# YaoFANGUK/video-subtitle-remover

Hardware: AMD Instinct MI355X
Metric: inpainted frames/sec @1080p (STTN, 5-frame window) (higher is better)
Workload: dtype f32; 1 GPU; 1080p synthetic clip, --inpaint-mode sttn-auto, 50-frame chunks resident in HBM, neighbor stride 5 / refs every 10 (BASELINE.json metric; model cost is resolution-independent); chunk_frames=50, parallelism=chunk-parallel x1, weights=synthetic variance-preserving (no checkpoint in the reference mount)

## Files before the change

### include/vsr_hip.h

```cpp
#ifndef VSR_HIP_H
#define VSR_HIP_H
#include <stdint.h>

#ifdef __cplusplus
extern "C" {
#endif

#define VSR_OK 0
#define VSR_ERR_ARG (-1)
#define VSR_ERR_STATE (-2)
#define VSR_ERR_HIP (-3)
#define VSR_ERR_NOGPU (-4)

#define VSR_VARIANT_STTN_AUTO 0
#define VSR_VARIANT_STTN_DET 1

typedef struct vsr_sttn vsr_sttn_t;
typedef struct vsr_plan vsr_plan_t;

int vsr_version(void);
const char* vsr_last_error(void);
int vsr_device_count(void);

int vsr_sttn_create(int variant, vsr_sttn_t** out);
// ... 304 lines not shown
    int32_t bufS, bufP;
    int64_t offS, offP, splitStride;
    int32_t M, N, ldS, ldP, nsplit;
    float scale;
} VsrSoftmaxInfo;

int vsr_plan_create(const vsr_sttn_t* h, int L, vsr_plan_t** out);
int vsr_plan_create_rows(const vsr_sttn_t* h, int L, int row_lo, int row_hi, vsr_plan_t** out);
int vsr_plan_create_box(const vsr_sttn_t* h, int L, int row_lo, int row_hi, int col_lo, int col_hi, vsr_plan_t** out);
int vsr_plan_create_ctx(const vsr_sttn_t* h, int L, int n_ctx, int row_lo, int row_hi, int col_lo, int col_hi, vsr_plan_t** out);
int vsr_raft_plan_create(const vsr_raft_t* h, int t, int H, int W, int iters, vsr_plan_t** out);
int vsr_rfc_plan_create(const vsr_rfc_t* h, int t, int H, int W, vsr_plan_t** out);
int vsr_pp_imgprop_plan_create(int t, int H, int W, vsr_plan_t** out);
int vsr_pp_gen_plan_create(const vsr_pp_t* h, int t, int lt, int H, int W, const uint8_t* window_flags, int nflags, vsr_plan_t** out);
int vsr_pp_gen_plan_create_mode(const vsr_pp_t* h, int t, int lt, int H, int W, const uint8_t* window_flags, int nflags, int row_lo, int row_hi,
                                int col_lo, int col_hi, int mode, vsr_plan_t** out);
int vsr_pp_gen_plan_create_box(const vsr_pp_t* h, int t, int lt, int H, int W, const uint8_t* window_flags, int nflags, int row_lo, int row_hi,
                               int col_lo, int col_hi, vsr_plan_t** out);
int vsr_lama_plan_create(const vsr_lama_t* h, int B, int H, int W, vsr_plan_t** out);
int64_t vsr_plan_consts(const vsr_plan_t* p, float* out, int64_t capacity);
void vsr_plan_destroy(vsr_plan_t* p);
int vsr_plan_num_buffers(const vsr_plan_t* p);
int64_t vsr_plan_buffer_elems(const vsr_plan_t* p, int buf);
int vsr_plan_num_tables(const vsr_plan_t* p);
int64_t vsr_plan_table_len(const vsr_plan_t* p, int t);
int vsr_plan_table_copy(const vsr_plan_t* p, int t, int32_t* out);
int vsr_plan_num_ops(const vsr_plan_t* p);
int vsr_plan_op(const vsr_plan_t* p, int i, VsrOpInfo* out);
int vsr_plan_op_lane(const vsr_plan_t* p, int i);
int vsr_plan_op_gemm(const vsr_plan_t* p, int i, int j, VsrGemmInfo* out);
int vsr_plan_op_softmax(const vsr_plan_t* p, int i, int j, VsrSoftmaxInfo* out);
int vsr_plan_counts(const vsr_plan_t* p, int32_t* counts);
double vsr_plan_flops(const vsr_plan_t* p);

#ifdef __cplusplus
}
#endif
#endif
```

### video-subtitle-remover_amd/_lib.py

```python
import ctypes as C
import os

_HERE = os.path.dirname(os.path.abspath(__file__))
LIB_PATH = os.path.join(_HERE, "lib", "libvsr_hip.so")

VSR_OK, VSR_ERR_ARG, VSR_ERR_STATE, VSR_ERR_HIP, VSR_ERR_NOGPU = 0, -1, -2, -3, -4
VARIANT = {"auto": 0, "det": 1}
BMODE_NK, BMODE_KN = 0, 1
ACT_NONE, ACT_LRELU02 = 0, 1
TILE_128x128, TILE_256x32, TILE_256x64, TILE_128x64 = 0, 1, 2, 3
TILE_256x128, TILE_256x256 = 4, 5
TILE_DIMS = {TILE_128x128: (128, 128), TILE_256x32: (256, 32), TILE_256x64: (256, 64), TILE_128x64: (128, 64), TILE_256x128: (256, 128), TILE_256x256: (256, 256)}


class VsrError(RuntimeError):
    def __init__(self, code, msg):
        super().__init__(f"libvsr_hip error {code}: {msg}")
        self.code = code


class GGProblem(C.Structure):
    _fields_ = [("A", C.c_void_p), ("B", C.c_void_p), ("C", C.c_void_p), ("bias", C.c_void_p), ("R", C.c_void_p),
                ("rowA", C.c_void_p), ("colA", C.c_void_p), ("rowB", C.c_void_p), ("colB", C.c_void_p),
                ("rowC", C.c_void_p), ("colC", C.c_void_p), ("rowR", C.c_void_p),
# ... 173 lines not shown
    "vsr_lama_packed_weights": (_L, [_P, _P, _L]),
    "vsr_lama_inpaint": (_I, [_P, _P, _L, _P, _L, _I, _I, _I, _P, _L, _P]),
    "vsr_lama_set_precision": (_I, [_P, _I]),
    "vsr_lama_fallbacks": (_L, [_P]),
    "vsr_lama_read_buffer": (_I, [_P, _I, _L, _L, _P]),
    "vsr_lama_flops": (_D, [_P, _I, _I, _I]),
    "vsr_lama_plan_create": (_I, [_P, _I, _I, _I, C.POINTER(_P)]),
    "vsr_telea_create": (_I, [C.POINTER(_P), _I, _I]),
    "vsr_telea_destroy": (None, [_P]),
    "vsr_telea_set_mask": (_I, [_P, _P, _I, _I]),
    "vsr_telea_plan_pixels": (_L, [_P]),
    "vsr_telea_plan_levels": (_I, [_P]),
    "vsr_telea_plan_taps": (_I, [_P]),
    "vsr_telea_plan_read": (_I, [_P, _P, _P, _P, _P]),
    "vsr_telea_plan_tmap": (_I, [_P, _P]),
    "vsr_telea_plan_weights": (_I, [_P, _P, _P]),
    "vsr_telea_inpaint": (_I, [_P, _P, _L, _I, _P]),
    "vsr_feather_alpha": (_I, [_P, _I, _I, _I, _P, _P]),
    "vsr_feather_composite": (_I, [_P, _L, _P, _L, _P, _I, _I, _I, _I, _P]),
    "vsr_plan_consts": (_L, [_P, _P, _L]),
    "vsr_plan_destroy": (None, [_P]),
    "vsr_plan_num_buffers": (_I, [_P]),
    "vsr_plan_buffer_elems": (_L, [_P, _I]),
    "vsr_plan_num_tables": (_I, [_P]),
    "vsr_plan_table_len": (_L, [_P, _I]),
    "vsr_plan_table_copy": (_I, [_P, _I, _P]),
    "vsr_plan_num_ops": (_I, [_P]),
    "vsr_plan_op": (_I, [_P, _I, C.POINTER(VsrOpInfo)]),
    "vsr_plan_op_lane": (_I, [_P, _I]),
    "vsr_plan_op_gemm": (_I, [_P, _I, _I, C.POINTER(VsrGemmInfo)]),
    "vsr_plan_op_softmax": (_I, [_P, _I, _I, C.POINTER(VsrSoftmaxInfo)]),
    "vsr_plan_counts": (_I, [_P, _P]),
    "vsr_plan_flops": (_D, [_P]),
    "vsr_switch_state": (_I, [C.c_char_p]),
    "vsr_flow_timing": (_I, [_I]),
    "vsr_flow_timing_reset": (_I, []),
    "vsr_flow_timing_get": (_I, [C.c_char_p, C.POINTER(C.c_double), C.POINTER(C.c_int64), C.POINTER(C.c_double)]),
    "vsr_flow_timing_keys": (C.c_int64, [_P, C.c_int64]),
}

if not os.path.exists(LIB_PATH):
    raise ImportError(
        f"{LIB_PATH} is missing: build the HIP extension first (__graft_entry__.build() or "
        f"`make -C {os.path.join(_HERE, 'csrc')}`); this package has no CPU fallback")

import torch

from . import switches

switches.export_defaults()
lib = C.CDLL(LIB_PATH)
for _name, (_res, _args) in SIGNATURES.items():
    _fn = getattr(lib, _name)
    _fn.restype = _res
    _fn.argtypes = _args


def last_error():
    return (lib.vsr_last_error() or b"").decode("utf-8", "replace")


def check(rc):
    if rc != 0:
        raise VsrError(rc, last_error())
    return rc
```

### video-subtitle-remover_amd/csrc/sttn_engine.hip

```cpp
#include <hip/hip_runtime.h>
#include <algorithm>
#include <math.h>
#include <stdio.h>
#include <stdlib.h>
#include <string.h>
#include <map>
#include <memory>
#include <string>
#include <utility>
#include <vector>
#include "../../include/vsr_hip.h"
#include "elementwise.h"
#include "gather_gemm.h"
#include "sttn_plan.h"

using namespace vsr;

static thread_local std::string g_err;
static int fail(int code, const std::string& msg)
{
    g_err = msg;
    return code;
}
int vsr_internal_fail(int code, const char* msg) { return fail(code, msg); }
// ... 9 lines not shown
        int rc_ = (expr);                                                                                  \
        if (rc_ != 0) return rc_;                                                                          \
    } while (0)

namespace {

struct OpDev {
    int kind = 0, tileCfg = 0, bmode = 0;
    const void* dDesc = nullptr;
    int nitems = 0, total = 0;
    int nQueues = 1;
    const void* dDesc7 = nullptr;
    int nitems7 = 0, total7 = 0;
    struct Vt { const float* B; const int32_t* rowB; const int32_t* colB; int K, N; int64_t ld; float* dst; };
    std::vector<Vt> vts;
    const void* src = nullptr;
    void* dst = nullptr;
    int H = 0, W = 0, C = 0, haloS = 0, haloD = 0, n = 0, ldy = 0, pix = 0, premask = 0;
    const int32_t* tFrameIdx = nullptr;
    const int32_t* tFirst = nullptr;
    const uint8_t* maskU8 = nullptr;
    const uint8_t* inU8 = nullptr;
    int M = 0, N = 0, nsplit = 0;
    int64_t splitStride = 0;
    const int32_t* tRowC = nullptr;
    const int32_t* tColC = nullptr;
    int rowLo = 0, rowHi = 0;
    int split = 0;
    bool aexp = false;
    bool thin = false;
    const float* lsum = nullptr;
    int ldL = 0;
    double flops = 0;
    int lane = 0;
    std::string tag;
};

struct PlanDev {
    std::unique_ptr<Plan> plan;
    uint64_t lastUse = 0;
    int32_t* dTables = nullptr;
    void* dDescs = nullptr;
    int32_t* dIsFloat = nullptr;
    unsigned int* dQueues = nullptr;
    int32_t* dTables7 = nullptr;
    float* dVt = nullptr;
    std::vector<OpDev> ops;
    ~PlanDev()
    {
        if (dTables7) (void)hipFree(dTables7);
        if (dVt) (void)hipFree(dVt);
        if (dQueues) (void)hipFree(dQueues);
        if (dTables) (void)hipFree(dTables);
        if (dDescs) (void)hipFree(dDescs);
        if (dIsFloat) (void)hipFree(dIsFloat);
    }
};

struct StripTables {
    void* dev = nullptr;
    const int32_t *dxofs, *dyofs, *uxofs, *uyofs;
    const int16_t *dialpha, *dibeta, *uialpha, *uibeta;
    const float *ufalpha, *ufbeta;
};

struct TimingRec {
    std::string tag, kernel;
    double flops;
    hipEvent_t a, b;
};

}

static bool sttn_thin(int precision, int bmode, const std::vector<GGProblem>& probs, int totalTiles);

struct vsr_sttn {
    Model model;
    int device = -1;
    bool finalized = false;
    void* bufs[BUF_COUNT] = {};
    int64_t cap[BUF_COUNT] = {};
    std::map<int64_t, std::unique_ptr<PlanDev>> plans;
    uint64_t useClock = 0;
    std::map<std::pair<int, int>, StripTables> strips;
    float* compAreas = nullptr;
    int64_t compAreasCap = 0;
    int32_t* dSel = nullptr;
    int dSelCap = 0;
    int precision = 0;
    float* weightsSplit = nullptr;
    unsigned int* dRangeFlag = nullptr;
    int64_t fallbacks = 0;
    int lanes = 2;
    hipStream_t laneStream[kMaxLanes] = {};
    hipEvent_t evFork = nullptr, evJoin[kMaxLanes] = {};
    std::vector<hipEvent_t> evDecode;
    int timing = 0;
    std::vector<TimingRec> pending;
    std::map<std::string, std::pair<double, std::pair<int, double>>> timed;
    explicit vsr_sttn(int variant) : model(variant)
    {
// ... 83 lines not shown
        if (kSlice < 256 || g.N < 32) return false;
        for (const GemmItem& o : op.gemm)
            if (anchorV7(op, o)) return true;
        return false;
    };
    std::vector<int64_t> vtLane(kMaxLanes, 0);
    int64_t tab7 = 0;
    for (const Op& op : P.ops) {
        if (op.kind != OP_GEMM || op.bmode != VSR_BMODE_KN) continue;
        int64_t sum = 0;
        for (const GemmItem& g : op.gemm)
            if (forV7(op, g)) { sum += (int64_t)g.N * g.K; tab7 += (g.N + 3) / 4 * 4; }
        if (sum > vtLane[op.lane]) vtLane[op.lane] = sum;
    }
    std::vector<int64_t> vtBase(kMaxLanes, 0);
    int64_t vtTotal = 0;
    for (int l = 0; l < kMaxLanes; ++l) { vtBase[l] = vtTotal; vtTotal += (vtLane[l] + 31) / 32 * 32; }
    if (vtTotal > 0) HIPCHK(hipMalloc((void**)&pd->dVt, (size_t)vtTotal * sizeof(float)));
    std::vector<int32_t> hostTab7((size_t)tab7, 0);
    if (tab7 > 0) HIPCHK(hipMalloc((void**)&pd->dTables7, (size_t)tab7 * sizeof(int32_t)));
    int64_t tab7Cursor = 0;
    size_t descBytes = 0;
    for (const Op& op : P.ops) {
        size_t n7 = 0;
        if (op.kind == OP_GEMM) for (const GemmItem& g : op.gemm) if (forV7(op, g)) ++n7;
        descBytes += ((op.gemm.size() + n7) * sizeof(GGProblem) + 63) / 64 * 64 + 64;
        descBytes += (op.softmax.size() * sizeof(SMProblem) + 63) / 64 * 64;
    }
    std::vector<char> hostDesc(descBytes + 64, 0);
    HIPCHK(hipMalloc(&pd->dDescs, descBytes + 64));
    size_t cursor = 0;
    for (const Op& op : P.ops) {
        OpDev od;
        od.kind = op.kind; od.tileCfg = op.tileCfg; od.bmode = op.bmode; od.flops = op.flops; od.tag = op.tag; od.lane = op.lane;
        if (op.kind == OP_GEMM) {
            std::vector<GGProblem> small, big;
            int64_t vtCursor = 0;
            for (size_t j = 0; j < op.gemm.size(); ++j) {
                const GemmItem& g = op.gemm[j];
                GGProblem q{};
                q.A = F(g.bufA, g.offA); q.B = F(g.bufB, g.offB); q.C = F(g.bufC, g.offC);
                if (fmt && g.bufB == BUF_WEIGHTS) q.B = h->weightsSplit + g.offB;
                q.bias = g.offBias >= 0 ? F(g.bufBias, g.offBias) : nullptr;
                q.R = g.bufR >= 0 ? F(g.bufR, g.offR) : nullptr;
                q.rowA = T(g.tRowA); q.colA = T(g.tColA); q.rowB = T(g.tRowB); q.colB = T(g.tColB);
                q.rowC = T(g.tRowC); q.colC = T(g.tColC); q.rowR = T(g.tRowR);
                q.M = g.M; q.N = g.N; q.K = g.K; q.tilesM = g.tilesM; q.tilesN = g.tilesN;
                q.splitK = g.splitK; q.chunksPerSplit = g.chunksPerSplit;
                q.act = g.act | ((fmt && !plainF32(g.bufC)) ? VSR_ACT_OUT_SPLIT : 0);
                q.alpha = g.alpha; q.splitStride = g.splitStride;
                if (forV7(op, g)) {
                    if (op.bmode == VSR_BMODE_KN) {
                        OpDev::Vt vt;
                        vt.B = q.B; vt.rowB = q.rowB; vt.colB = q.colB; vt.K = g.K; vt.N = g.N; vt.ld = g.K;
                        vt.dst = pd->dVt + vtBase[op.lane] + vtCursor;
                        vtCursor += (int64_t)g.N * g.K;
                        for (int n = 0; n < g.N; ++n) hostTab7[(size_t)(tab7Cursor + n)] = (int32_t)((int64_t)n * g.K);
                        q.B = vt.dst; q.rowB = pd->dTables7 + tab7Cursor; q.colB = q.colA;
                        tab7Cursor += (g.N + 3) / 4 * 4;
                        od.vts.push_back(vt);
                    }
                    GGProblem two[2];
                    const int n = vsr_v7_split(&q, cus, two);
                    for (int k = 0; k < n; ++k) big.push_back(two[k]);
                } else {
                    small.push_back(q);
                }
// ... 119 lines not shown
    const int prec = pd->plan->precision;
    const bool persistent = prec ? true : use_persistent();
    if (persistent) HIPCHK(hipMemsetAsync(pd->dQueues, 0, (pd->ops.size() + 1) * 16 * sizeof(unsigned int), stream));
    if (pd->plan->bufElems[BUF_ROWMAX] > 0)
        HIPCHK(hipMemsetAsync(h->bufs[BUF_ROWMAX], 0, (size_t)pd->plan->bufElems[BUF_ROWMAX] * sizeof(unsigned int), stream));
    const bool laned = pd->plan->lanes > 1;
    hipStream_t laneOf[kMaxLanes] = {stream, stream, stream, stream};
    if (laned) {
        if (!h->evFork) HIPCHK(hipEventCreateWithFlags(&h->evFork, hipEventDisableTiming));
        for (int l = 1; l < pd->plan->lanes; ++l) {
            if (!h->laneStream[l]) HIPCHK(hipStreamCreateWithFlags(&h->laneStream[l], hipStreamNonBlocking));
            if (!h->evJoin[l]) HIPCHK(hipEventCreateWithFlags(&h->evJoin[l], hipEventDisableTiming));
            laneOf[l] = h->laneStream[l];
        }
    }
    bool forked[kMaxLanes] = {};
    int lastDecodeLane = -1;
    size_t nDecode = 0;
    size_t opIndex = 0;
    for (const OpDev& od : pd->ops) {
        unsigned int* queue = persistent ? pd->dQueues + 16 * opIndex : nullptr;
        if (laned && (int)opIndex == pd->plan->firstWindowOp) HIPCHK(hipEventRecord(h->evFork, laneOf[0]));
        ++opIndex;
        hipStream_t const stream = laneOf[od.lane];
        if (laned && od.lane > 0 && !forked[od.lane]) {
            HIPCHK(hipStreamWaitEvent(stream, h->evFork, 0));
            forked[od.lane] = true;
        }
        if (laned && od.kind == OP_DECODE_OUT && lastDecodeLane >= 0 && lastDecodeLane != od.lane)
            HIPCHK(hipStreamWaitEvent(stream, h->evDecode[nDecode - 1], 0));
        TimingRec tr;
        const bool timed = h->timing == 1 || (h->timing == 2 && od.kind == OP_GEMM && od.tileCfg == VSR_TILE_128x64 && od.bmode == VSR_BMODE_NK && !od.thin);
        if (timed) {
            tr.tag = od.tag; tr.flops = od.flops;
            const bool big = od.kind == OP_GEMM && od.total7 > 0;
            tr.kernel = od.kind != OP_GEMM ? ("kernel:op:" + std::to_string(od.kind))
                      : (big && od.total == 0) ? ("kernel:gg:" + std::to_string(VSR_TILE_256x256) + ":0:v7")
                      : ("kernel:gg:" + std::to_string(od.tileCfg) + ":" + std::to_string(od.bmode) + ":v" +
                         std::to_string(od.thin ? 1 : gg_variant(od.bmode, prec)) + (od.aexp ? "x" : "") + (big ? "m" : ""));
            HIPCHK(hipEventCreate(&tr.a));
            HIPCHK(hipEventCreate(&tr.b));
            HIPCHK(hipEventRecord(tr.a, stream));
        }
        int rc = 0;
        static const bool qkSplit = [] { const char* e = getenv("VSR_F16_QK_SPLIT"); return e && atoi(e) == 1; }();
        const bool scoresSplit = prec == 3 && qkSplit && od.kind == OP_GEMM && od.tag == "attn.qk";
        switch (od.kind) {
        case OP_GEMM:
            for (const OpDev::Vt& vt : od.vts)
                if (rc == 0) rc = vsr_launch_kn_to_nk_split(vt.B, vt.rowB, vt.colB, vt.K, vt.N, vt.ld, vt.dst, stream);
            if (rc == 0 && od.total7 > 0)
                rc = vsr_launch_gather_gemm_dev((const GGProblem*)od.dDesc7, od.nitems7, od.total7, VSR_TILE_256x256, VSR_BMODE_NK, queue + 8,
                                                (prec == 3 && !scoresSplit) ? 6 : 5, 1, h->dRangeFlag, stream);
            if (rc == 0 && od.total > 0)
                rc = vsr_launch_gather_gemm_dev((const GGProblem*)od.dDesc, od.nitems, od.total, od.tileCfg, od.bmode, queue,
                                                (scoresSplit ? 5 : od.thin ? 1 : gg_variant(od.bmode, prec)) | (od.aexp ? VSR_VARIANT_A_EXP : 0), od.nQueues,
                                                prec ? h->dRangeFlag : nullptr, stream);
            break;
        case OP_SOFTMAX:
            rc = vsr_launch_softmax_dev((const SMProblem*)od.dDesc, od.nitems, od.total, stream);
            break;
        case OP_NORM_IM2COL:
            rc = vsr_launch_norm_im2col_fmt((const uint8_t*)od.src, od.H, od.W, od.n, (float*)od.dst, od.premask, od.maskU8, od.split, stream);
            break;
        case OP_UPSAMPLE2X:
            rc = vsr_launch_upsample2x_rows((const float*)od.src, od.H, od.W, od.C, od.haloS, (float*)od.dst, od.haloD, od.n, od.split,
                                            od.rowLo, od.rowHi > od.rowLo ? od.rowHi : 2 * od.H, stream);
// ... 21 lines not shown
        if (laned && od.kind == OP_DECODE_OUT) {
            if (h->evDecode.size() <= nDecode) {
                hipEvent_t e;
                HIPCHK(hipEventCreateWithFlags(&e, hipEventDisableTiming));
                h->evDecode.push_back(e);
            }
            HIPCHK(hipEventRecord(h->evDecode[nDecode], stream));
            lastDecodeLane = od.lane;
            ++nDecode;
        }
    }
    for (int l = 1; l < kMaxLanes; ++l)
        if (forked[l]) {
            HIPCHK(hipEventRecord(h->evJoin[l], laneOf[l]));
            HIPCHK(hipStreamWaitEvent(laneOf[0], h->evJoin[l], 0));
        }
    return 0;
}

static bool switch_rows_on() { static const bool v = [] { const char* e = getenv("VSR_DECODE_ROWS"); return !(e && atoi(e) == 0); }(); return v; }
static bool switch_cols_on() { static const bool v = [] { const char* e = getenv("VSR_DECODE_COLS"); return e && atoi(e) == 1; }(); return v; }

static int collect_timing(vsr_sttn* h, hipStream_t stream)
{
    if (h->pending.empty()) return 0;
    HIPCHK(hipStreamSynchronize(stream));
    for (TimingRec& tr : h->pending) {
        float ms = 0.f;
        HIPCHK(hipEventElapsedTime(&ms, tr.a, tr.b));
        for (const std::string* key : {&tr.tag, &tr.kernel}) {
            auto& acc = h->timed[*key];
            acc.first += ms;
            acc.second.first += 1;
            acc.second.second += tr.flops;
        }
        (void)hipEventDestroy(tr.a);
        (void)hipEventDestroy(tr.b);
    }
    h->pending.clear();
    return 0;
}

static int need_gpu(vsr_sttn* h)
{
    if (!h) return fail(VSR_ERR_ARG, "null handle");
    if (!h->finalized || h->device < 0)
        return fail(VSR_ERR_NOGPU, "model is not finalized on a HIP device (no GPU / finalize(device<0)); there is no CPU fallback");
    HIPCHK(hipSetDevice(h->device));
    return 0;
}

static int get_strip_tables(vsr_sttn* h, int W, int sh, StripTables** out)
{
    auto key = std::make_pair(W, sh);
    auto it = h->strips.find(key);
    if (it != h->strips.end()) { *out = &it->second; return 0; }
    const int mw = h->model.g.modelW, mh = h->model.g.modelH;
    std::vector<int32_t> dxo, dyo, uxo, uyo;
    std::vector<int16_t> dxa, dya, uxa, uya;
    std::vector<float> dxf, dyf, uxf, uyf;
    cv2_linear_tables(W, mw, true, dxo, dxa, dxf);
    cv2_linear_tables(sh, mh, false, dyo, dya, dyf);
    cv2_linear_tables(mw, W, true, uxo, uxa, uxf);
    cv2_linear_tables(mh, sh, false, uyo, uya, uyf);
    auto al = [](size_t v) { return (v + 15) / 16 * 16; };
    size_t o = 0;
    const size_t o_dxo = o; o += al(dxo.size() * 4);
// ... 493 lines not shown

double vsr_sttn_flops(vsr_sttn_t* h, int L)
{
    if (!h || !h->model.packed_ready() || L <= 0) { fail(VSR_ERR_ARG, "bad argument"); return -1.0; }
    try {
        Plan p(h->model, L);
        return p.flops;
    } catch (const std::exception& e) {
        fail(VSR_ERR_ARG, e.what());
        return -1.0;
    }
}

double vsr_sttn_flops_reference(vsr_sttn_t* h, int L)
{
    if (!h || !h->model.packed_ready() || L <= 0) { fail(VSR_ERR_ARG, "bad argument"); return -1.0; }
    try {
        Plan p(h->model, L);
        return p.refFlops;
    } catch (const std::exception& e) {
        fail(VSR_ERR_ARG, e.what());
        return -1.0;
    }
}

int vsr_switch_state(const char* name)
{
    if (!name) return -1;
    const std::string n(name);
    if (n == "VSR_DECODE_ROWS") return switch_rows_on() ? 1 : 0;
    if (n == "VSR_DECODE_COLS") return switch_cols_on() ? 1 : 0;
    if (n == "VSR_QKV0_SHARED") return Tuning::get(0).shareQkv0 ? 1 : 0;
    if (n == "VSR_TRIM_LAST_BLOCK") return Tuning::get(0).trimLastBlock ? 1 : 0;
    return -1;
}

int vsr_sttn_timing(vsr_sttn_t* h, int enable)
{
    if (!h) return fail(VSR_ERR_ARG, "null handle");
    h->timing = enable < 0 ? 0 : (enable > 2 ? 1 : enable);
    return 0;
}

int vsr_sttn_timing_reset(vsr_sttn_t* h)
{
    if (!h) return fail(VSR_ERR_ARG, "null handle");
    h->timed.clear();
    return 0;
}

int vsr_sttn_timing_get(vsr_sttn_t* h, const char* prefix, double* total_ms, int32_t* launches, double* flops)
{
    if (!h || !prefix) return fail(VSR_ERR_ARG, "bad argument");
    double ms = 0, fl = 0;
    int n = 0;
    const size_t pl = strlen(prefix);
    for (const auto& kv : h->timed)
        if (kv.first.compare(0, pl, prefix) == 0) { ms += kv.second.first; n += kv.second.second.first; fl += kv.second.second.second; }
    if (total_ms) *total_ms = ms;
    if (launches) *launches = n;
    if (flops) *flops = fl;
    return 0;
}

static void tile_dims(int cfg, int& BM, int& BN)
{
// ... 252 lines not shown
int vsr_plan_op_lane(const vsr_plan_t* p, int i) { return (p && i >= 0 && i < (int)p->plan->ops.size()) ? p->plan->ops[i].lane : -1; }

int vsr_plan_op_gemm(const vsr_plan_t* p, int i, int j, VsrGemmInfo* o)
{
    if (!p || !o || i < 0 || i >= (int)p->plan->ops.size()) return fail(VSR_ERR_ARG, "bad op");
    const Op& op = p->plan->ops[i];
    if (op.kind != OP_GEMM || j < 0 || j >= (int)op.gemm.size()) return fail(VSR_ERR_ARG, "bad gemm item");
    const GemmItem& g = op.gemm[j];
    o->bufA = g.bufA; o->bufB = g.bufB; o->bufC = g.bufC; o->bufR = g.bufR;
    o->offA = g.offA; o->offB = g.offB; o->offC = g.offC; o->offR = g.offR; o->offBias = g.offBias;
    o->tRowA = g.tRowA; o->tColA = g.tColA; o->tRowB = g.tRowB; o->tColB = g.tColB; o->tRowC = g.tRowC;
    o->tColC = g.tColC; o->tRowR = g.tRowR;
    o->M = g.M; o->N = g.N; o->K = g.K; o->tilesM = g.tilesM; o->tilesN = g.tilesN; o->splitK = g.splitK;
    o->chunksPerSplit = g.chunksPerSplit; o->splitStride = g.splitStride; o->alpha = g.alpha; o->act = g.act;
    return 0;
}
int vsr_plan_op_softmax(const vsr_plan_t* p, int i, int j, VsrSoftmaxInfo* o)
{
    if (!p || !o || i < 0 || i >= (int)p->plan->ops.size()) return fail(VSR_ERR_ARG, "bad op");
    const Op& op = p->plan->ops[i];
    if (op.kind != OP_SOFTMAX || j < 0 || j >= (int)op.softmax.size()) return fail(VSR_ERR_ARG, "bad softmax item");
    const SoftmaxItem& s = op.softmax[j];
    o->bufS = s.bufS; o->bufP = s.bufP; o->offS = s.offS; o->offP = s.offP; o->splitStride = s.splitStride;
    o->M = s.M; o->N = s.N; o->ldS = s.ldS; o->ldP = s.ldP; o->nsplit = s.nsplit; o->scale = s.scale;
    return 0;
}
int vsr_plan_counts(const vsr_plan_t* p, int32_t* counts)
{
    if (!p || !counts) return fail(VSR_ERR_ARG, "bad argument");
    memcpy(counts, p->plan->compCount.data(), p->plan->compCount.size() * sizeof(int32_t));
    return 0;
}
double vsr_plan_flops(const vsr_plan_t* p) { return p ? p->plan->flops : -1.0; }

}
```

### video-subtitle-remover_amd/csrc/sttn_plan.cpp

```cpp
#include "sttn_plan.h"
#include "gather_gemm.h"
#include <assert.h>
#include <math.h>
#include <stdexcept>
#include <stdlib.h>

namespace vsr {

static int envInt(const char* name, int dflt)
{
    const char* v = getenv(name);
    return (v && *v) ? atoi(v) : dflt;
}

const Tuning& Tuning::get(int precision)
{
    static const Tuning t[2] = {
        [] {
            Tuning x;
            x.convTile = envInt("VSR_CONV_TILE", VSR_TILE_128x64);
            if (x.convTile == VSR_TILE_256x128) x.convTile = VSR_TILE_128x64;
            x.qkTile = envInt("VSR_QK_TILE", VSR_TILE_128x64);
            x.qkvTile = envInt("VSR_QKV_TILE", x.convTile);
            x.pvTile = envInt("VSR_PV_TILE", VSR_TILE_128x64);
            x.pvSplitChunks = envInt("VSR_PV_SPLIT_CHUNKS", 50);
            x.convChannelMajor = envInt("VSR_CONV_KORDER", 1);
            x.fuseSoftmax = envInt("VSR_FUSE_SOFTMAX", 1) && envInt("VSR_GG_VARIANT", 3) == 3 && envInt("VSR_PV_VARIANT", 1) == 1;
            x.outConvBlocked = envInt("VSR_OUT_CONV_BLOCKED", 1);
            x.trimLastBlock = envInt("VSR_TRIM_LAST_BLOCK", 1);
            x.shareQkv0 = envInt("VSR_QKV0_SHARED", 0);
            return x;
        }(),
        [] {
            Tuning x;
            x.convTile = envInt("VSR_CONV_TILE", VSR_TILE_128x64);
            x.qkTile = envInt("VSR_QK_TILE", VSR_TILE_128x64);
            x.qkvTile = envInt("VSR_QKV_TILE", x.convTile);
            x.pvTile = envInt("VSR_PV_TILE", VSR_TILE_128x64);
            x.pvSplitChunks = envInt("VSR_PV_SPLIT_CHUNKS", 50);
            x.convChannelMajor = envInt("VSR_CONV_KORDER", 1);
            x.fuseSoftmax = 0;
            x.outConvBlocked = envInt("VSR_OUT_CONV_BLOCKED", 1);
            x.trimLastBlock = envInt("VSR_TRIM_LAST_BLOCK", 1);
            x.shareQkv0 = envInt("VSR_QKV0_SHARED", 0);
            return x;
        }()};
    return t[precision ? 1 : 0];
}

static inline int cdiv(int a, int b) { return (a + b - 1) / b; }
static inline int64_t rup(int64_t a, int64_t b) { return (a + b - 1) / b * b; }

Geometry Geometry::make(int variant)
{
    Geometry g{};
    g.variant = variant;
    g.channels = 256;
    g.blocks = 8;
    g.nscales = 4;
    g.neighborStride = 5;
    g.refLength = 10;
    if (variant == 0) {
        g.modelW = 640; g.modelH = 120;
        const int pw[4] = {80, 32, 10, 5}, ph[4] = {15, 6, 5, 3};
        for (int i = 0; i < 4; ++i) { g.patchW[i] = pw[i]; g.patchH[i] = ph[i]; }
    } else {
        g.modelW = 432; g.modelH = 240;
        const int pw[4] = {108, 36, 18, 9}, ph[4] = {60, 20, 10, 5};
        for (int i = 0; i < 4; ++i) { g.patchW[i] = pw[i]; g.patchH[i] = ph[i]; }
    }
    g.featW = g.modelW / 4;
    g.featH = g.modelH / 4;
    return g;
}

Model::Model(int variant) : g(Geometry::make(variant)) { blk.resize(g.blocks); }

// ... 239 lines not shown
                v.push_back((int32_t)o);
            }
    const int32_t first = v.empty() ? 0 : v[0];
    while ((int64_t)v.size() % padTo) v.push_back(first);
    return table(key, std::move(v));
}

int PlanBuilder::tColsConvHW(const Act& a, int kh, int kw, int dil, int c0, int cin)
{
    if (cin < 0) cin = a.C - c0;
    const std::string key = "CC:" + std::to_string(a.halo) + ":" + std::to_string(a.W) + ":" + std::to_string(a.C) +
                            ":" + std::to_string(kh) + "x" + std::to_string(kw) + ":" + std::to_string(dil) + ":" +
                            std::to_string(c0) + ":" + std::to_string(cin);
    auto it = tableKey_.find(key);
    if (it != tableKey_.end()) return it->second;
    if (a.halo < dil * (kh / 2) || a.halo < dil * (kw / 2)) throw std::runtime_error("activation halo too small for conv");
    if (cin % VSR_GG_KC || c0 % VSR_GG_KC) throw std::runtime_error("conv input channels must be a multiple of 32");
    std::vector<int32_t> v;
    auto off = [&](int ky, int kx, int c) {
        return (int32_t)(((int64_t)(ky - kh / 2) * dil * a.Wp() + (kx - kw / 2) * dil) * a.C + c0 + c);
    };
    if (Tuning::get().convChannelMajor) {
        for (int c = 0; c < cin; c += VSR_GG_KC)
            for (int ky = 0; ky < kh; ++ky)
                for (int kx = 0; kx < kw; ++kx) v.push_back(off(ky, kx, c));
    } else {
        for (int ky = 0; ky < kh; ++ky)
            for (int kx = 0; kx < kw; ++kx)
                for (int c = 0; c < cin; c += VSR_GG_KC) v.push_back(off(ky, kx, c));
    }
    return table(key, std::move(v));
}

int PlanBuilder::tRowsLinear(int count, int ld, int padTo)
{
    const std::string key = "RL:" + std::to_string(count) + ":" + std::to_string(ld) + ":" + std::to_string(padTo);
    auto it = tableKey_.find(key);
    if (it != tableKey_.end()) return it->second;
    std::vector<int32_t> v;
    for (int i = 0; i < count; ++i) { checkFits((int64_t)i * ld); v.push_back((int32_t)((int64_t)i * ld)); }
    while ((int)v.size() % padTo) v.push_back(0);
    return table(key, std::move(v));
}

int PlanBuilder::tColsLinear(int nchunks, int padTo)
{
    const std::string key = "CL:" + std::to_string(nchunks) + ":" + std::to_string(padTo);
    auto it = tableKey_.find(key);
    if (it != tableKey_.end()) return it->second;
    std::vector<int32_t> v;
    for (int i = 0; i < nchunks; ++i) v.push_back(i * VSR_GG_KC);
    while ((int)v.size() < padTo) v.push_back(0);
    return table(key, std::move(v));
}

int Plan::tRowsTokens(int T, int s, int choff, int count, int padTo, int oy0, int oy1, int ox0, int ox1, const std::vector<int>* fids)
{
    const int pw = g.patchW[s], ph = g.patchH[s], ow = g.featW / pw, oh = g.featH / ph, C3 = 3 * g.channels;
    if (oy1 < 0) oy1 = oh;
    if (ox1 < 0) ox1 = ow;
    std::string key = "RT:" + std::to_string(T) + ":" + std::to_string(s) + ":" + std::to_string(choff) + ":" +
                      std::to_string(count) + ":" + std::to_string(padTo) + ":" + std::to_string(oy0) + "-" + std::to_string(oy1) +
                      ":" + std::to_string(ox0) + "-" + std::to_string(ox1);
    if (fids) key += ":f" + idsKey(std::vector<int>(fids->begin(), fids->begin() + T));
    auto it = tableKey_.find(key);
    if (it != tableKey_.end()) return it->second;
// ... 61 lines not shown
    for (int y = 0; y < ph; ++y)
        for (int x = 0; x < pw; ++x)
            for (int c0 = 0; c0 < dk; c0 += VSR_GG_KC) v.push_back((int32_t)(((int64_t)y * a.Wp() + x) * a.C + c0));
    while ((int)v.size() < padTo) v.push_back(0);
    return table(key, std::move(v));
}

static std::vector<int> iota(int n)
{
    std::vector<int> v(n);
    for (int i = 0; i < n; ++i) v[i] = i;
    return v;
}

void Plan::addConv(const char* tag, const Act& in, const std::vector<int>& inIds, const Act& out, int nOut, int ksz,
                   int stride, int dil, const ConvW& w, int act, const Act* res, const std::vector<int>* resIds, int ylo, int yhi,
                   int xlo, int xhi)
{
    if (yhi < 0) yhi = out.H;
    if (xhi < 0) xhi = out.W;
    if (ylo < 0 || yhi > out.H || ylo >= yhi || (stride != 1 && (ylo != 0 || yhi != out.H))) throw std::runtime_error(std::string("conv row range: ") + tag);
    if (xlo < 0 || xhi > out.W || xlo >= xhi || (stride != 1 && (xlo != 0 || xhi != out.W))) throw std::runtime_error(std::string("conv column range: ") + tag);
    const bool rect = xlo != 0 || xhi != out.W;
    const int oh = yhi - ylo, ow = xhi - xlo;
    if (w.K != ksz * ksz * in.C) throw std::runtime_error(std::string("conv K mismatch: ") + tag);
    if ((int)inIds.size() != nOut) throw std::runtime_error("conv frame list mismatch");
    Op op;
    op.kind = OP_GEMM;
    op.tag = tag;
    op.bmode = VSR_BMODE_NK;
    op.tileCfg = pickTile(w.cout);
    int BM, BN;
    tileDims(op.tileCfg, BM, BN);
    GemmItem it{};
    it.M = nOut * oh * ow;
    it.N = w.cout;
    it.K = w.K;
    it.tilesM = cdiv(it.M, BM);
    it.tilesN = cdiv(it.N, BN);
    it.splitK = 1;
    it.chunksPerSplit = it.K / VSR_GG_KC;
    it.splitStride = 0;
    it.alpha = 1.f;
    it.act = act;
    it.bufA = in.buf; it.offA = 0;
    it.tRowA = rect ? tRowsActRect(in, inIds, ylo, yhi, xlo, xhi, BM) : tRowsAct(in, inIds, oh, out.W, stride, BM, (int64_t)ylo * in.Wp() * in.C);
    it.tColA = tColsConv(in, ksz, dil);
    it.bufB = BUF_WEIGHTS; it.offB = w.w;
    it.tRowB = tRowsLinear(it.N, it.K, BN);
    it.tColB = tColsLinear(it.K / VSR_GG_KC, it.K / VSR_GG_KC);
    it.bufC = out.buf; it.offC = 0;
    it.tRowC = rect ? tRowsActRect(out, iota(nOut), ylo, yhi, xlo, xhi, BM) : tRowsAct(out, iota(nOut), oh, out.W, 1, BM, (int64_t)ylo * out.Wp() * out.C);
    it.tColC = tColsLinear(cdiv(it.N, VSR_GG_KC), it.tilesN * BN / VSR_GG_KC);
    it.offBias = w.b;
    if (res) {
        it.bufR = res->buf; it.offR = 0;
        it.tRowR = rect ? tRowsActRect(*res, *resIds, ylo, yhi, xlo, xhi, BM) : tRowsAct(*res, *resIds, oh, out.W, 1, BM, (int64_t)ylo * res->Wp() * res->C);
    } else {
        it.bufR = -1; it.offR = 0; it.tRowR = -1;
    }
    op.flops = 2.0 * it.M * it.N * (double)(ksz * ksz * in.C);
    op.gemm.push_back(it);
    need(out.buf, (int64_t)nOut * out.frameElems());
    flops += op.flops;
    ops.push_back(std::move(op));
}

void Plan::addAttention(int Tq, int T, const BlockW&, int attLo, int attHi, int attXLo, int attXHi, int qkvBuf, const std::vector<int>* fids, int qFirst)
{
    std::vector<int> qf;
    for (int t = 0; t < Tq; ++t) qf.push_back(fids ? (*fids)[qFirst + t] : qFirst + t);
    const std::vector<int>* qfids = qFirst > 0 ? &qf : fids;
    if (qkvBuf < 0) qkvBuf = lb(BUF_QKV);
    if (attHi < 0) attHi = g.featH;
    if (attXHi < 0) attXHi = g.featW;
    const Tuning& tu = tu_;
    const int C = g.channels, dk = C / g.nscales;
    const Act att{lb(BUF_ATT), T, g.featH, g.featW, C, 1};
    Op qk, sm, pv;
    qk.kind = OP_GEMM; qk.tag = "attn.qk"; qk.tileCfg = tu.qkTile; qk.bmode = VSR_BMODE_NK;
    sm.kind = OP_SOFTMAX; sm.tag = "attn.softmax";
    pv.kind = OP_GEMM; pv.tag = "attn.pv"; pv.tileCfg = tu.pvTile; pv.bmode = VSR_BMODE_KN;
    int qBM, qBN, pBM, pBN;
    tileDims(qk.tileCfg, qBM, qBN);
    tileDims(pv.tileCfg, pBM, pBN);
    std::vector<Op> reduces;
    bool pvFused = false;
    int64_t sOff = 0, pOff = 0, partOff = 0, lOff = 0;
    for (int s = g.nscales - 1; s >= 0; --s) {
        const int pw = g.patchW[s], ph = g.patchH[s];
        const int Pn = (g.featW / pw) * (g.featH / ph);
        const int Ntok = T * Pn;
        const int oy0 = attLo / ph, oy1 = cdiv(attHi, ph);
        const int ox0 = attXLo / pw, ox1 = cdiv(attXHi, pw);
        const int Mtok = Tq * (oy1 - oy0) * (ox1 - ox0);
// ... 426 lines not shown
        it.bufC = BUF_QKV0; it.offC = 0;
        it.tRowC = tRowsLinear(it.M, 3 * C, BM);
        it.tColC = tColsLinear(it.N / VSR_GG_KC, it.tilesN * BN / VSR_GG_KC);
        it.offBias = bw.qkv.b;
        it.bufR = -1; it.tRowR = -1;
        op.flops = 2.0 * it.M * (double)it.N * it.K;
        flops += op.flops;
        trimmedFlops_ -= op.flops;
        op.gemm.push_back(it);
        need(BUF_QKV0, (int64_t)it.M * 3 * C);
        ops.push_back(std::move(op));
    }

    std::vector<int32_t> visits(L, 0);
    const int ns = g.neighborStride;
    for (int f = 0; f < L; f += ns) {
        std::vector<int> neighbors, refs;
        for (int i = (f - ns > 0 ? f - ns : 0); i < (f + ns + 1 < L ? f + ns + 1 : L); ++i) neighbors.push_back(i);
        for (int i = 0; i < L; i += g.refLength) {
            bool inN = false;
            for (int n : neighbors) inN |= (n == i);
            if (!inN) refs.push_back(i);
        }
        if (neighbors.back() < nCtx) continue;
        lane_ = nwindows % lanes;
        const size_t first = ops.size();
        if (firstWindowOp < 0) firstWindowOp = (int)first;
        buildWindow(neighbors, refs, visits);
        for (size_t i = first; i < ops.size(); ++i) ops[i].lane = lane_;
    }
    lane_ = 0;
    compCount = visits;
    refFlops = flops + trimmedFlops_;
    if (nCtx > 0) refFlops = Plan(model, L_, precision_, 1, decLo_, decHi_, decXLo_, decXHi_).refFlops;
}

void cv2_linear_tables(int ssize, int dsize, bool clampX, std::vector<int32_t>& ofs, std::vector<int16_t>& icoef,
                       std::vector<float>& fcoef)
{
    const double inv_scale = (double)dsize / (double)ssize;
    const double scale = 1.0 / inv_scale;
    ofs.resize(dsize);
    icoef.resize(2 * (size_t)dsize);
    fcoef.resize(2 * (size_t)dsize);
    for (int d = 0; d < dsize; ++d) {
        float f = (float)((d + 0.5) * scale - 0.5);
        int s = (int)floorf(f);
        f -= (float)s;
        if (clampX) {
            if (s < 0) { f = 0.f; s = 0; }
            if (s >= ssize - 1) { f = 0.f; s = ssize - 1; }
        }
        ofs[d] = s;
        const float c0 = 1.f - f, c1 = f;
        fcoef[2 * d] = c0;
        fcoef[2 * d + 1] = c1;
        auto sat = [](float v) {
            long r = lrintf(v * 2048.f);
            if (r > 32767) r = 32767;
            if (r < -32768) r = -32768;
            return (int16_t)r;
        };
        icoef[2 * d] = sat(c0);
        icoef[2 * d + 1] = sat(c1);
    }
}
// ... 3 lines not shown
```

### video-subtitle-remover_amd/csrc/sttn_plan.h

```cpp
#pragma once
#include <stdint.h>
#include <map>
#include <string>
#include <vector>

namespace vsr {

struct Geometry {
    int variant;
    int modelW, modelH;
    int featW, featH;
    int channels;
    int blocks;
    int nscales;
    int patchW[4], patchH[4];
    int neighborStride;
    int refLength;
    static Geometry make(int variant);
};

struct Tuning {
    int convTile;
    int qkTile;
    int qkvTile;
    int pvTile;
    int pvSplitChunks;
    int convChannelMajor;
    int outConvBlocked;
    int shareQkv0;
    int trimLastBlock;
    int fuseSoftmax;
    static const Tuning& get(int precision = 0);
};

struct ConvW {
    int64_t w = -1, b = -1;
    int cout = 0, K = 0;
};
struct BlockW { ConvW qkv, out, ffn1, ffn2; };

class Model {
public:
    explicit Model(int variant);
    bool set_param(const std::string& name, const float* data, const int64_t* shape, int ndim, std::string& err);
    bool pack(std::string& err);
    bool packed_ready() const { return ready_; }
    Geometry g;
    ConvW enc[4], dec[4];
    ConvW dec4blk;
    static constexpr int kOutBlkH = 2, kOutBlkW = 4;
    std::vector<BlockW> blk;
    std::vector<float> packed;
    static std::vector<std::string> expected_keys(int variant);
private:
    struct Raw { std::vector<float> v; std::vector<int64_t> shape; };
    std::map<std::string, Raw> raw_;
    bool ready_ = false;
    bool pack_conv(const std::string& key, ConvW& cw, int cinPad, std::string& err);
    bool pack_conv_blocked(const std::string& key, ConvW& cw, int bh, int bw, std::string& err);
};

enum BufId {
    BUF_WEIGHTS = 0, BUF_IN_U8, BUF_IM2COL, BUF_E1, BUF_E2, BUF_E3, BUF_FEATS, BUF_X0, BUF_X1, BUF_QKV,
    BUF_S, BUF_P, BUF_ATT, BUF_F1, BUF_UP1, BUF_D1, BUF_D2, BUF_UP2, BUF_D3, BUF_D4, BUF_COMP, BUF_PVPART, BUF_MASK_U8,
// ... 18 lines not shown

enum OpKind { OP_NORM_IM2COL = 0, OP_GEMM = 1, OP_SOFTMAX = 2, OP_UPSAMPLE2X = 3, OP_DECODE_OUT = 4, OP_REDUCE_SCATTER = 5,
              OP_EW = 6  };

struct GemmItem {
    int bufA, bufB, bufC, bufR;
    int64_t offA, offB, offC, offR, offBias;
    int tRowA, tColA, tRowB, tColB, tRowC, tColC, tRowR;
    int M, N, K;
    int tilesM, tilesN, splitK, chunksPerSplit;
    int64_t splitStride;
    float alpha;
    int act;
    int bufBias;
};
struct SoftmaxItem {
    int bufS, bufP;
    int64_t offS, offP, splitStride;
    int M, N, ldS, ldP, nsplit;
    float scale;
};
struct Op {
    int kind = 0;
    int tileCfg = 0, bmode = 0;
    std::vector<GemmItem> gemm;
    std::vector<SoftmaxItem> softmax;
    int bufSrc = -1, bufDst = -1, H = 0, W = 0, C = 0, haloS = 0, haloD = 0, n = 0;
    int ldy = 0, pix = 0, tFrameIdx = -1, tFirst = -1;
    int premask = 0;
    int bufMask = -1;
    int M = 0, N = 0, nsplit = 0, tRowC = -1, tColC = -1;
    int64_t offSrc = 0, offDst = 0, splitStride = 0;
    double flops = 0;
    int lane = 0;
    std::string tag;
    int ew = 0;
    int ibuf[4] = {-1, -1, -1, -1};
    int64_t ioff[4] = {0, 0, 0, 0};
    int ipar[16] = {0, 0, 0, 0, 0, 0, 0, 0, 0, 0, 0, 0, 0, 0, 0, 0};
    float fpar[4] = {0.f, 0.f, 0.f, 0.f};
};

struct Act {
    int buf, n, H, W, C, halo;
    int Hp() const { return H + 2 * halo; }
    int Wp() const { return W + 2 * halo; }
    int64_t frameElems() const { return (int64_t)Hp() * Wp() * C; }
    int64_t pix(int f, int y, int x) const { return (((int64_t)f * Hp() + y + halo) * Wp() + x + halo) * C; }
    int64_t elems() const { return (int64_t)n * frameElems(); }
};

constexpr int BUF_PLAN_CONST = -2;

struct PlanIR {
    std::vector<int64_t> bufElems;
    std::vector<float> consts;
    std::vector<std::vector<int32_t>> tables;
    std::vector<Op> ops;
    std::vector<int32_t> compCount;
    double flops = 0;
    double refFlops = 0;
    virtual ~PlanIR() {}
};

class PlanBuilder : public PlanIR {
protected:
    std::map<std::string, int> tableKey_;
    int table(const std::string& key, std::vector<int32_t>&& v);
    int tRowsAct(const Act& a, const std::vector<int>& ids, int oh, int ow, int stride, int padTo, int64_t add);
    int tRowsActRect(const Act& a, const std::vector<int>& ids, int ylo, int yhi, int xlo, int xhi, int padTo);
    int tColsConvHW(const Act& a, int kh, int kw, int dil, int c0 = 0, int cin = -1);
    int tColsConv(const Act& a, int ksz, int dil) { return tColsConvHW(a, ksz, ksz, dil); }
    int tRowsLinear(int count, int ld, int padTo);
    int tColsLinear(int nchunks, int padTo);
    void need(int buf, int64_t elems);
};

class Plan : public PlanBuilder {
public:
    Plan(const Model& model, int L, int precision = 0, int lanes = 1, int decLo = 0, int decHi = 0, int decXLo = 0, int decXHi = 0, int nCtx = 0);
    static void decoder_bounds(const Geometry& g, int precision, int decLo, int decHi, int decXLo, int decXHi, int* lo, int* hi, int* xlo, int* xhi);
    int decLo = 0, decHi = 0;
    int decXLo = 0, decXHi = 0;
    int L;
    int nCtx = 0;
    int precision;
    int lanes;
    int firstWindowOp = -1;
    Geometry g;
    int nwindows = 0;
private:
    const Model& m_;
    const Tuning& tu_;
    int lane_ = 0;
    bool qkv0_ = false;
    int lb(int buf) const { return laneBuf(buf, lane_); }
    int64_t rowmaxElems_ = 0;
    double trimmedFlops_ = 0;
    int pickTile(int N) const;
    int tRowsTokens(int T, int s, int choff, int count, int padTo, int oy0 = 0, int oy1 = -1, int ox0 = 0, int ox1 = -1,
                    const std::vector<int>* fids = nullptr);
    int tColsPatch(int s, int padTo);
    int tRowsTokensAct(const Act& a, int T, int s, int padTo, int oy0 = 0, int oy1 = -1, int ox0 = 0, int ox1 = -1);
    int tColsPatchAct(const Act& a, int s, int padTo);
    void addConv(const char* tag, const Act& in, const std::vector<int>& inIds, const Act& out, int nOut,
// ... 16 lines not shown
```

### video-subtitle-remover_amd/switches.py

```python
import os

DEFAULTS = {"VSR_DECODE_COLS": "1", "VSR_PP_DECODE_BOX": "1", "VSR_PP_ENC_CACHE": "1", "VSR_QKV0_SHARED": "1"}


def export_defaults():
    for k, v in DEFAULTS.items():
        os.environ.setdefault(k, v)


LIBRARY_SIDE = ("VSR_DECODE_COLS", "VSR_QKV0_SHARED")


def on(name):
    if name in LIBRARY_SIDE:
        from . import _lib

        v = _lib.lib.vsr_switch_state(name.encode())
        if v >= 0:
            return v == 1
    return os.environ.get(name, DEFAULTS[name]) == "1"
```

Measured before the change: 220.2 frames/s.

## Skip zero-padding conv taps on top/bottom border rows via split GEMM items

For 3x3 stride-1 convolutions, the output rows are split into a middle band using all nine taps and top/bottom border bands that omit the taps reading only zero-padded halo rows. This shrinks K for the border bands and uses new gather tables for the reduced activation and weight columns. It removes wasted multiply-adds on padding, at the cost of more, smaller GEMM items per op with possible tile underutilization. Executed-FLOP accounting is added for timing reports.

```diff
diff --git a/include/vsr_hip.h b/include/vsr_hip.h
--- a/include/vsr_hip.h
+++ b/include/vsr_hip.h
@@ -360,6 +360,7 @@
 int vsr_plan_op_softmax(const vsr_plan_t* p, int i, int j, VsrSoftmaxInfo* out);
 int vsr_plan_counts(const vsr_plan_t* p, int32_t* counts);
 double vsr_plan_flops(const vsr_plan_t* p);
+double vsr_plan_flops_executed(const vsr_plan_t* p);
 
 #ifdef __cplusplus
 }
diff --git a/video-subtitle-remover_amd/_lib.py b/video-subtitle-remover_amd/_lib.py
--- a/video-subtitle-remover_amd/_lib.py
+++ b/video-subtitle-remover_amd/_lib.py
@@ -229,6 +229,7 @@
     "vsr_plan_op_softmax": (_I, [_P, _I, _I, C.POINTER(VsrSoftmaxInfo)]),
     "vsr_plan_counts": (_I, [_P, _P]),
     "vsr_plan_flops": (_D, [_P]),
+    "vsr_plan_flops_executed": (_D, [_P]),
     "vsr_switch_state": (_I, [C.c_char_p]),
     "vsr_flow_timing": (_I, [_I]),
     "vsr_flow_timing_reset": (_I, []),
diff --git a/video-subtitle-remover_amd/csrc/sttn_engine.hip b/video-subtitle-remover_amd/csrc/sttn_engine.hip
--- a/video-subtitle-remover_amd/csrc/sttn_engine.hip
+++ b/video-subtitle-remover_amd/csrc/sttn_engine.hip
@@ -65,6 +65,7 @@
     const float* lsum = nullptr;
     int ldL = 0;
     double flops = 0;
+    double flopsExec = 0;
     int lane = 0;
     std::string tag;
 };
@@ -99,7 +100,7 @@
 
 struct TimingRec {
     std::string tag, kernel;
-    double flops;
+    double flops, flopsExec;
     hipEvent_t a, b;
 };
 
@@ -249,7 +250,7 @@
     size_t cursor = 0;
     for (const Op& op : P.ops) {
         OpDev od;
-        od.kind = op.kind; od.tileCfg = op.tileCfg; od.bmode = op.bmode; od.flops = op.flops; od.tag = op.tag; od.lane = op.lane;
+        od.kind = op.kind; od.tileCfg = op.tileCfg; od.bmode = op.bmode; od.flops = op.flops; od.flopsExec = op.flopsExecuted >= 0 ? op.flopsExecuted : op.flops; od.tag = op.tag; od.lane = op.lane;
         if (op.kind == OP_GEMM) {
             std::vector<GGProblem> small, big;
             int64_t vtCursor = 0;
@@ -435,7 +436,7 @@
         TimingRec tr;
         const bool timed = h->timing == 1 || (h->timing == 2 && od.kind == OP_GEMM && od.tileCfg == VSR_TILE_128x64 && od.bmode == VSR_BMODE_NK && !od.thin);
         if (timed) {
-            tr.tag = od.tag; tr.flops = od.flops;
+            tr.tag = od.tag; tr.flops = od.flops; tr.flopsExec = od.flopsExec;
             const bool big = od.kind == OP_GEMM && od.total7 > 0;
             tr.kernel = od.kind != OP_GEMM ? ("kernel:op:" + std::to_string(od.kind))
                       : (big && od.total == 0) ? ("kernel:gg:" + std::to_string(VSR_TILE_256x256) + ":0:v7")
@@ -523,7 +524,7 @@
             auto& acc = h->timed[*key];
             acc.first += ms;
             acc.second.first += 1;
-            acc.second.second += tr.flops;
+            acc.second.second += key == &tr.kernel ? tr.flopsExec : tr.flops;
         }
         (void)hipEventDestroy(tr.a);
         (void)hipEventDestroy(tr.b);
@@ -1083,6 +1084,7 @@
     if (n == "VSR_DECODE_COLS") return switch_cols_on() ? 1 : 0;
     if (n == "VSR_QKV0_SHARED") return Tuning::get(0).shareQkv0 ? 1 : 0;
     if (n == "VSR_TRIM_LAST_BLOCK") return Tuning::get(0).trimLastBlock ? 1 : 0;
+    if (n == "VSR_SKIP_PAD_TAPS") return Tuning::get(0).skipPadTaps ? 1 : 0;
     return -1;
 }
 
@@ -1401,5 +1403,6 @@
     return 0;
 }
 double vsr_plan_flops(const vsr_plan_t* p) { return p ? p->plan->flops : -1.0; }
-
-}
+double vsr_plan_flops_executed(const vsr_plan_t* p) { return !p ? -1.0 : (p->plan->flopsExecuted >= 0 ? p->plan->flopsExecuted : p->plan->flops); }
+
+}
diff --git a/video-subtitle-remover_amd/csrc/sttn_plan.cpp b/video-subtitle-remover_amd/csrc/sttn_plan.cpp
--- a/video-subtitle-remover_amd/csrc/sttn_plan.cpp
+++ b/video-subtitle-remover_amd/csrc/sttn_plan.cpp
@@ -1,5 +1,6 @@
 #include "sttn_plan.h"
 #include "gather_gemm.h"
+#include <algorithm>
 #include <assert.h>
 #include <math.h>
 #include <stdexcept>
@@ -29,6 +30,7 @@
             x.outConvBlocked = envInt("VSR_OUT_CONV_BLOCKED", 1);
             x.trimLastBlock = envInt("VSR_TRIM_LAST_BLOCK", 1);
             x.shareQkv0 = envInt("VSR_QKV0_SHARED", 0);
+            x.skipPadTaps = envInt("VSR_SKIP_PAD_TAPS", 1);
             return x;
         }(),
         [] {
@@ -43,6 +45,7 @@
             x.outConvBlocked = envInt("VSR_OUT_CONV_BLOCKED", 1);
             x.trimLastBlock = envInt("VSR_TRIM_LAST_BLOCK", 1);
             x.shareQkv0 = envInt("VSR_QKV0_SHARED", 0);
+            x.skipPadTaps = envInt("VSR_SKIP_PAD_TAPS", 1);
             return x;
         }()};
     return t[precision ? 1 : 0];
@@ -348,6 +351,33 @@
     return table(key, std::move(v));
 }
 
+int PlanBuilder::tColsConvTaps(const Act& a, int dil, unsigned taps)
+{
+    const std::string key = "CT:" + std::to_string(a.halo) + ":" + std::to_string(a.W) + ":" + std::to_string(a.C) + ":" +
+                            std::to_string(dil) + ":" + std::to_string(taps);
+    auto it = tableKey_.find(key);
+    if (it != tableKey_.end()) return it->second;
+    if (a.halo < dil) throw std::runtime_error("activation halo too small for conv");
+    if (a.C % VSR_GG_KC) throw std::runtime_error("conv input channels must be a multiple of 32");
+    std::vector<int32_t> v;
+    for (int c = 0; c < a.C; c += VSR_GG_KC)
+        for (int tap = 0; tap < 9; ++tap)
+            if (taps >> tap & 1) v.push_back((int32_t)(((int64_t)(tap / 3 - 1) * dil * a.Wp() + (tap % 3 - 1) * dil) * a.C + c));
+    return table(key, std::move(v));
+}
+
+int PlanBuilder::tColsWeightTaps(int cin, unsigned taps)
+{
+    const std::string key = "CW:" + std::to_string(cin) + ":" + std::to_string(taps);
+    auto it = tableKey_.find(key);
+    if (it != tableKey_.end()) return it->second;
+    std::vector<int32_t> v;
+    for (int c = 0; c < cin; c += VSR_GG_KC)
+        for (int tap = 0; tap < 9; ++tap)
+            if (taps >> tap & 1) v.push_back((c / VSR_GG_KC * 9 + tap) * VSR_GG_KC);
+    return table(key, std::move(v));
+}
+
 int PlanBuilder::tRowsLinear(int count, int ld, int padTo)
 {
     const std::string key = "RL:" + std::to_string(count) + ":" + std::to_string(ld) + ":" + std::to_string(padTo);
@@ -475,35 +505,54 @@
     op.tileCfg = pickTile(w.cout);
     int BM, BN;
     tileDims(op.tileCfg, BM, BN);
-    GemmItem it{};
-    it.M = nOut * oh * ow;
-    it.N = w.cout;
-    it.K = w.K;
-    it.tilesM = cdiv(it.M, BM);
-    it.tilesN = cdiv(it.N, BN);
-    it.splitK = 1;
-    it.chunksPerSplit = it.K / VSR_GG_KC;
-    it.splitStride = 0;
-    it.alpha = 1.f;
-    it.act = act;
-    it.bufA = in.buf; it.offA = 0;
-    it.tRowA = rect ? tRowsActRect(in, inIds, ylo, yhi, xlo, xhi, BM) : tRowsAct(in, inIds, oh, out.W, stride, BM, (int64_t)ylo * in.Wp() * in.C);
-    it.tColA = tColsConv(in, ksz, dil);
-    it.bufB = BUF_WEIGHTS; it.offB = w.w;
-    it.tRowB = tRowsLinear(it.N, it.K, BN);
-    it.tColB = tColsLinear(it.K / VSR_GG_KC, it.K / VSR_GG_KC);
-    it.bufC = out.buf; it.offC = 0;
-    it.tRowC = rect ? tRowsActRect(out, iota(nOut), ylo, yhi, xlo, xhi, BM) : tRowsAct(out, iota(nOut), oh, out.W, 1, BM, (int64_t)ylo * out.Wp() * out.C);
-    it.tColC = tColsLinear(cdiv(it.N, VSR_GG_KC), it.tilesN * BN / VSR_GG_KC);
-    it.offBias = w.b;
-    if (res) {
-        it.bufR = res->buf; it.offR = 0;
-        it.tRowR = rect ? tRowsActRect(*res, *resIds, ylo, yhi, xlo, xhi, BM) : tRowsAct(*res, *resIds, oh, out.W, 1, BM, (int64_t)ylo * res->Wp() * res->C);
+    auto item = [&](int y0, int y1, unsigned taps) {
+        const int rows = y1 - y0;
+        int ntaps = 0;
+        for (int t = 0; t < ksz * ksz; ++t) ntaps += taps >> t & 1;
+        const bool all = ntaps == ksz * ksz;
+        GemmItem it{};
+        it.M = nOut * rows * ow;
+        it.N = w.cout;
+        it.K = all ? w.K : ntaps * in.C;
+        it.tilesM = cdiv(it.M, BM);
+        it.tilesN = cdiv(it.N, BN);
+        it.splitK = 1;
+        it.chunksPerSplit = it.K / VSR_GG_KC;
+        it.splitStride = 0;
+        it.alpha = 1.f;
+        it.act = act;
+        it.bufA = in.buf; it.offA = 0;
+        it.tRowA = rect ? tRowsActRect(in, inIds, y0, y1, xlo, xhi, BM) : tRowsAct(in, inIds, rows, out.W, stride, BM, (int64_t)y0 * in.Wp() * in.C);
+        it.tColA = all ? tColsConv(in, ksz, dil) : tColsConvTaps(in, dil, taps);
+        it.bufB = BUF_WEIGHTS; it.offB = w.w;
+        it.tRowB = tRowsLinear(it.N, w.K, BN);
+        it.tColB = all ? tColsLinear(it.K / VSR_GG_KC, it.K / VSR_GG_KC) : tColsWeightTaps(in.C, taps);
+        it.bufC = out.buf; it.offC = 0;
+        it.tRowC = rect ? tRowsActRect(out, iota(nOut), y0, y1, xlo, xhi, BM) : tRowsAct(out, iota(nOut), rows, out.W, 1, BM, (int64_t)y0 * out.Wp() * out.C);
+        it.tColC = tColsLinear(cdiv(it.N, VSR_GG_KC), it.tilesN * BN / VSR_GG_KC);
+        it.offBias = w.b;
+        if (res) {
+            it.bufR = res->buf; it.offR = 0;
+            it.tRowR = rect ? tRowsActRect(*res, *resIds, y0, y1, xlo, xhi, BM) : tRowsAct(*res, *resIds, rows, out.W, 1, BM, (int64_t)y0 * res->Wp() * res->C);
+        } else {
+            it.bufR = -1; it.offR = 0; it.tRowR = -1;
+        }
+        op.gemm.push_back(it);
+    };
+    const int H = out.H;
+    if (tu_.skipPadTaps && tu_.convChannelMajor && ksz == 3 && stride == 1 && in.H == H && H >= 2 * dil) {
+        const int topHi = yhi < dil ? yhi : dil, botLo = ylo > H - dil ? ylo : H - dil;
+        const int midLo = ylo > dil ? ylo : dil, midHi = yhi < H - dil ? yhi : H - dil;
+        if (midHi > midLo) item(midLo, midHi, 0x1ff);
+        if (topHi > ylo) item(ylo, topHi, 0x1f8);
+        if (yhi > botLo) item(botLo, yhi, 0x03f);
+        std::stable_sort(op.gemm.begin(), op.gemm.end(), [](const GemmItem& a, const GemmItem& b) { return (int64_t)a.M * a.K > (int64_t)b.M * b.K; });
     } else {
-        it.bufR = -1; it.offR = 0; it.tRowR = -1;
-    }
-    op.flops = 2.0 * it.M * it.N * (double)(ksz * ksz * in.C);
-    op.gemm.push_back(it);
+        item(ylo, yhi, (1u << (ksz * ksz)) - 1);
+    }
+    op.flops = 2.0 * nOut * oh * ow * (double)w.cout * (double)(ksz * ksz * in.C);
+    op.flopsExecuted = 0;
+    for (const GemmItem& it : op.gemm) op.flopsExecuted += 2.0 * it.M * (double)it.N * it.K;
     need(out.buf, (int64_t)nOut * out.frameElems());
     flops += op.flops;
     ops.push_back(std::move(op));
@@ -996,6 +1045,8 @@
     lane_ = 0;
     compCount = visits;
     refFlops = flops + trimmedFlops_;
+    flopsExecuted = 0;
+    for (const Op& op : ops) flopsExecuted += op.flopsExecuted >= 0 ? op.flopsExecuted : op.flops;
     if (nCtx > 0) refFlops = Plan(model, L_, precision_, 1, decLo_, decHi_, decXLo_, decXHi_).refFlops;
 }
 
diff --git a/video-subtitle-remover_amd/csrc/sttn_plan.h b/video-subtitle-remover_amd/csrc/sttn_plan.h
--- a/video-subtitle-remover_amd/csrc/sttn_plan.h
+++ b/video-subtitle-remover_amd/csrc/sttn_plan.h
@@ -30,6 +30,7 @@
     int shareQkv0;
     int trimLastBlock;
     int fuseSoftmax;
+    int skipPadTaps;
     static const Tuning& get(int precision = 0);
 };
 
@@ -114,6 +115,7 @@
     int M = 0, N = 0, nsplit = 0, tRowC = -1, tColC = -1;
     int64_t offSrc = 0, offDst = 0, splitStride = 0;
     double flops = 0;
+    double flopsExecuted = -1;
     int lane = 0;
     std::string tag;
     int ew = 0;
@@ -141,6 +143,7 @@
     std::vector<Op> ops;
     std::vector<int32_t> compCount;
     double flops = 0;
+    double flopsExecuted = -1;
     double refFlops = 0;
     virtual ~PlanIR() {}
 };
@@ -153,6 +156,8 @@
     int tRowsActRect(const Act& a, const std::vector<int>& ids, int ylo, int yhi, int xlo, int xhi, int padTo);
     int tColsConvHW(const Act& a, int kh, int kw, int dil, int c0 = 0, int cin = -1);
     int tColsConv(const Act& a, int ksz, int dil) { return tColsConvHW(a, ksz, ksz, dil); }
+    int tColsConvTaps(const Act& a, int dil, unsigned taps);
+    int tColsWeightTaps(int cin, unsigned taps);
     int tRowsLinear(int count, int ld, int padTo);
     int tColsLinear(int nchunks, int padTo);
     void need(int buf, int64_t elems);
diff --git a/video-subtitle-remover_amd/switches.py b/video-subtitle-remover_amd/switches.py
--- a/video-subtitle-remover_amd/switches.py
+++ b/video-subtitle-remover_amd/switches.py
@@ -1,6 +1,6 @@
 import os
 
-DEFAULTS = {"VSR_DECODE_COLS": "1", "VSR_PP_DECODE_BOX": "1", "VSR_PP_ENC_CACHE": "1", "VSR_QKV0_SHARED": "1"}
+DEFAULTS = {"VSR_DECODE_COLS": "1", "VSR_PP_DECODE_BOX": "1", "VSR_PP_ENC_CACHE": "1", "VSR_QKV0_SHARED": "1", "VSR_SKIP_PAD_TAPS": "1"}
 
 
 def export_defaults():
@@ -8,7 +8,7 @@
         os.environ.setdefault(k, v)
 
 
-LIBRARY_SIDE = ("VSR_DECODE_COLS", "VSR_QKV0_SHARED")
+LIBRARY_SIDE = ("VSR_DECODE_COLS", "VSR_QKV0_SHARED", "VSR_SKIP_PAD_TAPS")
 
 
 def on(name):
```

Result: faster. 223.4 frames/s, median of 6 (+1.5%).
